# RaphaelHaddad/Real-Time-Brain-Inspired-Video-Memory

Measured on NVIDIA B200. Metric: queries_per_sec_top10_384d, higher is better.
Workload: dtype tf32

## Files before the change

### real-time-brain-inspired-video-memory_b200/csrc/common.cuh

```cuda
#pragma once
#include <cuda_runtime.h>
#include <cuda_bf16.h>
#include <stdint.h>
#include <stdio.h>
#include <math.h>
#include <utility>
#include "../../include/vidmem.h"

namespace vm {

void set_error(const char *fmt, ...);
#define VM_CUDA_CHECK(expr)                                                                      \
    do {                                                                                         \
        cudaError_t _e = (expr);                                                                 \
        if (_e != cudaSuccess) {                                                                 \
            vm::set_error("%s failed: %s (%s:%d)", #expr, cudaGetErrorString(_e), __FILE__, __LINE__); \
            return VM_ERR_CUDA;                                                                  \
        }                                                                                        \
    } while (0)
#define VM_REQUIRE(cond, code, ...)          \
    do {                                     \
        if (!(cond)) {                       \
            vm::set_error(__VA_ARGS__);      \
            return (code);                   \
        }                                    \
    } while (0)

__device__ __forceinline__ void pdl_wait() { asm volatile("griddepcontrol.wait;" ::: "memory"); }
__device__ __forceinline__ void pdl_launch_dependents() { asm volatile("griddepcontrol.launch_dependents;" ::: "memory"); }

template <typename... KArgs, typename... Args>
static inline cudaError_t launch_pdl(void (*kernel)(KArgs...), dim3 grid, dim3 block, size_t smem, cudaStream_t st, bool pdl,
                                     Args &&...args)
{
    cudaLaunchConfig_t cfg = {};
    cfg.gridDim = grid; cfg.blockDim = block; cfg.dynamicSmemBytes = smem; cfg.stream = st;
    cudaLaunchAttribute at[1];
    at[0].id = cudaLaunchAttributeProgrammaticStreamSerialization;
    at[0].val.programmaticStreamSerializationAllowed = 1;
    cfg.attrs = at;
    cfg.numAttrs = pdl ? 1 : 0;
    return cudaLaunchKernelEx(&cfg, kernel, std::forward<Args>(args)...);
}

template <auto Kernel>
static inline cudaError_t max_smem_once(int bytes)
{
    static bool set[64] = {};
    int dev = 0;
    cudaError_t e = cudaGetDevice(&dev);
    if (e != cudaSuccess || set[dev & 63]) return e;
    e = cudaFuncSetAttribute(Kernel, cudaFuncAttributeMaxDynamicSharedMemorySize, bytes);
    if (e == cudaSuccess) set[dev & 63] = true;
    return e;
}

__host__ __device__ __forceinline__ uint32_t f32_ordered(float f)
{
#ifdef __CUDA_ARCH__
    uint32_t b = __float_as_uint(f);
#else
    uint32_t b;
    memcpy(&b, &f, 4);
#endif
    return (b & 0x80000000u) ? ~b : (b | 0x80000000u);
}
__host__ __device__ __forceinline__ float f32_from_ordered(uint32_t o)
{
    uint32_t b = (o & 0x80000000u) ? (o & 0x7FFFFFFFu) : ~o;
#ifdef __CUDA_ARCH__
    return __uint_as_float(b);
#else
    float f;
    memcpy(&f, &b, 4);
    return f;
#endif
}
__host__ __device__ __forceinline__ uint64_t make_key(float score, uint32_t row)
{
    return ((uint64_t)f32_ordered(score) << 32) | (uint64_t)(0xFFFFFFFFu - row);
}
__host__ __device__ __forceinline__ uint32_t key_row(uint64_t k) { return 0xFFFFFFFFu - (uint32_t)(k & 0xFFFFFFFFu); }
// ... 210 lines not shown
```

### real-time-brain-inspired-video-memory_b200/csrc/scan_tc.cu

```cuda
#include "tc_common.cuh"

namespace vm {
using namespace tc;

static constexpr int TC_BLOCK_M = 128;
static constexpr int TC_STAGE_BYTES = TC_BLOCK_M * 128;
static constexpr int TC_ACC = 8;
static constexpr int TC_THREADS_SVC = 288;
static constexpr int TC_THREADS = 192;
static constexpr int TC_TMEM_COLS = 512;
static constexpr int TC_MAX_STAGES = 8;

struct CollectArgs {
    const float *thr;
    uint64_t *buf;
    int *cnt;
    int cap;
    const int *pending;
};

struct BandArgs {
    uint64_t *slab;
    int *scnt;
    uint64_t *ubuf;
// ... 15 lines not shown
    const int es = dtype == VM_F32 ? 4 : 2;
    L.nq_pad = (nq + 15) & ~15;
    L.KB = (ld * es + 127) / 128;
    L.split = (split && dtype == VM_BF16) ? 1 : 0;
    uint32_t o = 0;
    L.off_b = o; o += (uint32_t)L.KB * L.nq_pad * 128 * (L.split ? 2 : 1);
    const uint32_t epi = (uint32_t)L.nq_pad * (4 + 4 + 4 + 16) + 64 + 8 * (2 * TC_MAX_STAGES + 1 + 2 * TC_ACC) + 16;
    int64_t room = 227 * 1024 - 2048 - (int64_t)o - epi;
    L.stages = (int)(room / TC_STAGE_BYTES);
    if (L.stages > TC_MAX_STAGES) L.stages = TC_MAX_STAGES;
    if (L.stages < 0) L.stages = 0;
    L.off_a = o; o += (uint32_t)L.stages * TC_STAGE_BYTES;
    L.off_tauf = o; o += (uint32_t)L.nq_pad * 4;
    L.off_lcnt = o; o += (uint32_t)L.nq_pad * 4;
    L.off_cmax = o; o += (uint32_t)L.nq_pad * 4;
    L.off_wmax = o; o += (uint32_t)L.nq_pad * 16;
    L.off_flags = o; o += 64;
    L.off_bars = o; o += 8 * (2 * TC_MAX_STAGES + 1 + 2 * TC_ACC);
    L.off_tmem = o; o += 16;
    L.total = o + 1024;
#ifdef VIDMEM_AB_SMEMPAD
    if (L.total < 220 * 1024) L.total = 220 * 1024;
#endif
    return L;
}

__device__ __forceinline__ uint32_t own_kth_score(const uint64_t *slab, int n, int k, int lane)
{
    constexpr int PER = SCAN_SLAB / 32;
    uint32_t vals[PER];
#pragma unroll
    for (int t = 0; t < PER; ++t) {
        const int i = lane + 32 * t;
        vals[t] = i < n ? (uint32_t)(__ldcg(slab + i) >> 32) : 0u;
    }
    uint32_t prefix = 0;
    int need = k;
    for (int bit = 31; bit >= 12; --bit) {
        const uint32_t hi = bit == 31 ? 0u : (0xFFFFFFFFu << (bit + 1));
        int cnt = 0;
#pragma unroll
        for (int t = 0; t < PER; ++t) cnt += ((vals[t] & hi) == prefix && ((vals[t] >> bit) & 1u)) ? 1 : 0;
        const int tot = __reduce_add_sync(0xffffffffu, cnt);
        if (tot >= need) prefix |= 1u << bit;
        else need -= tot;
    }
    int ge = 0;
#pragma unroll
    for (int t = 0; t < PER; ++t) ge += (vals[t] != 0u && vals[t] >= prefix) ? 1 : 0;
    ge = __reduce_add_sync(0xffffffffu, ge);
    return (ge >= k && prefix != 0u) ? prefix : 0u;
}

template <bool TF32, bool DUMP, bool SPLIT>
__global__ void __launch_bounds__(DUMP ? TC_THREADS : TC_THREADS_SVC, 1)
scan_tc_kernel(const __grid_constant__ CUtensorMap tmA, const __grid_constant__ CUtensorMap tmB,
               const float *__restrict__ inv_norms, int64_t n, int num_tiles, int nq, TcLayout L, uint64_t *__restrict__ dump_keys,
               uint32_t *__restrict__ seed_tab, int *__restrict__ seed_ctr, CollectArgs col, BandArgs ub, int svc_sleep)
{
    const bool collect = !DUMP && col.thr != nullptr;
#ifndef VIDMEM_AB_NOPDL
    pdl_launch_dependents();
#endif
    if (collect) {
        pdl_wait();
        if (*col.pending == 0) return;
    }

    extern __shared__ __align__(16) uint8_t smem_raw[];
    uint8_t *base = smem_raw + ((1024u - (smem_u32(smem_raw) & 1023u)) & 1023u);
    uint8_t *sB = base + L.off_b;
    uint8_t *sA = base + L.off_a;
    float *tauf = (float *)(base + L.off_tauf);
    int *lcnt = (int *)(base + L.off_lcnt);
    uint32_t *cmax = (uint32_t *)(base + L.off_cmax);
    uint32_t *wmax = (uint32_t *)(base + L.off_wmax);
    volatile int *s_done = (volatile int *)(base + L.off_flags);
    uint64_t *bars = (uint64_t *)(base + L.off_bars);
    uint64_t *full = bars, *empty = bars + TC_MAX_STAGES, *qfull = bars + 2 * TC_MAX_STAGES;
    uint64_t *tfull = qfull + 1, *tempty = tfull + TC_ACC;
    uint32_t *tmem_slot = (uint32_t *)(base + L.off_tmem);

    const int warp = __shfl_sync(0xffffffffu, threadIdx.x >> 5, 0);
    const int lane = threadIdx.x & 31;
    const int nq_pad = L.nq_pad, KB = L.KB, stages = L.stages;
    constexpr int ELEMS = TF32 ? 32 : 64;

    if (warp == 0 && lane == 0) {
        tma_prefetch_desc(&tmA);
        tma_prefetch_desc(&tmB);
        for (int s = 0; s < stages; ++s) { mbar_init(&full[s], 1); mbar_init(&empty[s], 1); }
        mbar_init(qfull, 1);
        for (int a = 0; a < TC_ACC; ++a) { mbar_init(&tfull[a], 1); mbar_init(&tempty[a], 4); }
        fence_barrier_init();
    }
    if (warp == 1) tmem_alloc(tmem_slot, TC_TMEM_COLS);
#ifndef VIDMEM_AB_NOPDL
    if (!collect) pdl_wait();
#endif
    if (warp >= 2 && warp < 6) {
        const int e = threadIdx.x - 64;
        if (e < nq_pad) {
            lcnt[e] = 0;
            cmax[e] = 0u;
            tauf[e] = collect ? (e < nq ? col.thr[e] : INFINITY) : (e < nq ? -INFINITY : INFINITY);
        }
        if (e < 2) s_done[e] = 0;
    }
    tc_fence_before();
    __syncthreads();
    tc_fence_after();
    const uint32_t tmem_base = *tmem_slot;
    uint32_t *gbound = seed_tab ? seed_tab + SEED_TAB_WORDS : nullptr;

    if (warp == 0) {
        if (elect_one()) {
            constexpr int QPARTS = SPLIT ? 2 : 1;
            mbar_arrive_expect_tx(qfull, (uint32_t)(KB * QPARTS) * nq_pad * 128);
            for (int part = 0; part < QPARTS; ++part)
                for (int kb = 0; kb < KB; ++kb)
                    tma_load_2d(&tmB, qfull, sB + (size_t)(part * KB + kb) * nq_pad * 128, kb * ELEMS, part * nq_pad, L2_EVICT_LAST);
        }
        __syncwarp();
        int stage = 0;
        uint32_t phase = 0;
        for (int tile = blockIdx.x; tile < num_tiles; tile += gridDim.x) {
            for (int kb = 0; kb < KB; ++kb) {
                mbar_wait(&empty[stage], phase ^ 1);
                if (elect_one()) {
                    mbar_arrive_expect_tx(&full[stage], TC_STAGE_BYTES);
                    tma_load_2d(&tmA, &full[stage], sA + (size_t)stage * TC_STAGE_BYTES, kb * ELEMS, tile * TC_BLOCK_M, L2_EVICT_FIRST);
                }
                __syncwarp();
                if (++stage == stages) { stage = 0; phase ^= 1; }
            }
        }
    } else if (warp == 1) {
        const uint32_t idesc = make_idesc(TF32 ? 2u : 1u, TC_BLOCK_M, (uint32_t)nq_pad);
        mbar_wait(qfull, 0);
        tc_fence_after();
        int stage = 0, acc = 0;
        uint32_t phase = 0, acc_phase = 0;
        const uint64_t da0 = make_smem_desc_sw128(smem_u32(sA)), db0 = make_smem_desc_sw128(smem_u32(sB));
        const uint32_t kb_step = (uint32_t)(nq_pad * 128) >> 4, lo_step = (uint32_t)(KB * nq_pad * 128) >> 4;
        for (int tile = blockIdx.x; tile < num_tiles; tile += gridDim.x) {
            mbar_wait(&tempty[acc], acc_phase ^ 1);
            tc_fence_after();
            const uint32_t d_tmem = tmem_base + (uint32_t)(acc * nq_pad);
            for (int kb = 0; kb < KB; ++kb) {
                mbar_wait(&full[stage], phase);
                tc_fence_after();
                if (elect_one()) {
                    const uint64_t da = da0 + (uint64_t)((uint32_t)stage * (TC_STAGE_BYTES >> 4));
                    const uint64_t db = db0 + (uint64_t)((uint32_t)kb * kb_step);
#pragma unroll
                    for (int j = 0; j < 4; ++j) {
                        umma<TF32>(d_tmem, da + 2 * j, db + 2 * j, idesc, (uint32_t)((kb | j) != 0));
                        if constexpr (SPLIT) umma<TF32>(d_tmem, da + 2 * j, db + lo_step + 2 * j, idesc, 1u);
                    }
                    umma_commit(&empty[stage]);
                    if (kb == KB - 1) umma_commit(&tfull[acc]);
                }
                __syncwarp();
                if (++stage == stages) { stage = 0; phase ^= 1; }
            }
            if (++acc == TC_ACC) { acc = 0; acc_phase ^= 1; }
        }
    } else if (warp < 6) {
        const int e = threadIdx.x - 64;
        const int quad = warp & 3;
        const int row_in_tile = quad * 32 + lane;
        int acc = 0;
        uint32_t acc_phase = 0;
        if constexpr (DUMP) {
            for (int tile = blockIdx.x; tile < num_tiles; tile += gridDim.x) {
                const int64_t r = (int64_t)tile * TC_BLOCK_M + row_in_tile;
                const float iv = r < n ? __ldg(inv_norms + r) : -1.0f;
                mbar_wait(&tfull[acc], acc_phase);
                tc_fence_after();
                const uint32_t taddr = tmem_base + ((uint32_t)(quad * 32) << 16) + (uint32_t)(acc * nq_pad);
                uint64_t *out = dump_keys + (int64_t)tile * nq * TC_BLOCK_M + row_in_tile;
                for (int c = 0; c < nq_pad; c += 16) {
                    uint32_t v[16];
                    tmem_ld16(taddr + c, v);
                    tmem_ld_wait();
#pragma unroll
                    for (int j = 0; j < 16; ++j)
                        if (c + j < nq)
                            out[(int64_t)(c + j) * TC_BLOCK_M] = iv >= 0.0f ? make_key(__uint_as_float(v[j]) * iv, (uint32_t)r) : 0ull;
                }
                tc_fence_before();
                __syncwarp();
                if (lane == 0) mbar_arrive(&tempty[acc]);
                if (++acc == TC_ACC) { acc = 0; acc_phase ^= 1; }
            }
        } else {
        if (ub.use_seed && !collect) {
            const int64_t row0 = (int64_t)blockIdx.x * TC_BLOCK_M + row_in_tile;
            const float inv0 = row0 < n ? __ldg(inv_norms + row0) : -1.0f;
            mbar_wait(&tfull[0], 0);
            tc_fence_after();
            const uint32_t taddr0 = tmem_base + ((uint32_t)(quad * 32) << 16);
            for (int c = 0; c < nq_pad; c += 16) {
                uint32_t v[16];
                tmem_ld16(taddr0 + c, v);
// ... 87 lines not shown
                            if (key == 1) tauf[q] = 0.0f;
                            continue;
#endif
                            const int pos = atomicAdd(&lcnt[q], 1);
                            atomicMax(&cmax[q], (uint32_t)(key >> 32));
                            if (pos < SCAN_SLAB) __stcg(my_slab + (size_t)q * SCAN_SLAB + pos, key);
                            else {
                                const int p = atomicAdd(ub.ucnt + q, 1);
                                if (p < ub.ucap) __stcg(ub.ubuf + (size_t)q * ub.ucap + p, key);
                                else tauf[q] = INFINITY;
                            }
                        }
                    }
                }
            };
            uint32_t va[16], vb[16];
#ifdef VIDMEM_AB_NOEPI
            if (tile < 0)
#endif
            tmem_ld16(taddr, va);
#ifdef VIDMEM_AB_NOEPI
            if (tile < 0)
#endif
            for (int c = 0; c < nq_pad; c += 32) {
                tmem_ld_wait();
                if (c + 16 < nq_pad) tmem_ld16(taddr + c + 16, vb);
                process(va, c);
                if (c + 16 < nq_pad) {
                    tmem_ld_wait();
                    if (c + 32 < nq_pad) tmem_ld16(taddr + c + 32, va);
                    process(vb, c + 16);
                }
            }
#ifdef VIDMEM_AB_TILEBAR
            named_bar_sync(1, 128);
#endif
            tc_fence_before();
            __syncwarp();
            if (lane == 0) mbar_arrive(&tempty[acc]);
            if (++acc == TC_ACC) { acc = 0; acc_phase ^= 1; }
            row = row_next;
            inv = inv_next;
        }
        if (!collect) {
            named_bar_sync(1, 128);
            if (e < nq) {
                ub.scnt[(size_t)blockIdx.x * nq + e] = lcnt[e];
                if (seed_tab != nullptr) __stcg(seed_tab + (size_t)blockIdx.x * nq_pad + e, cmax[e]);
            }
        }
        }
        __syncwarp();
        if (lane == 0) atomicAdd((int *)s_done, 1);
    } else {
#ifdef VIDMEM_AB_NOSVC
        if (false) {
#else
        if (!DUMP && warp == 8 && seed_tab != nullptr && !collect) {
#endif
            const int G = (int)gridDim.x;
            while (s_done[1] == 0 && s_done[0] < 4) __nanosleep(100);
            uint32_t pub0 = 0xFFFFFFFFu, pub1 = 0xFFFFFFFFu;
            uint32_t kth_done = 0;
            const uint64_t *my_slab = ub.slab + (size_t)blockIdx.x * nq * SCAN_SLAB;
            while (!__any_sync(0xffffffffu, s_done[0] >= 4)) {
#pragma unroll
                for (int h = 0; h < 2; ++h) {
                    const int q = lane + 32 * h;
                    if (q < nq) {
                        const uint32_t c = *(volatile uint32_t *)(cmax + q);
                        uint32_t &pub = h ? pub1 : pub0;
                        if (c != pub && c != 0u) { __stcg(seed_tab + (size_t)blockIdx.x * nq_pad + q, c); pub = c; }
                    }
                }
                __syncwarp();
                if (G >= ub.ksel)
                    for (int q = blockIdx.x; q < nq; q += G) {
                        const float sd = seed_select(seed_tab, G, nq_pad, q, ub.ksel, lane);
                        if (lane == 0 && sd > -INFINITY) atomicMax(gbound + q, f32_ordered(sd));
                    }
                __syncwarp();
#ifndef VIDMEM_AB_KTH_LEVELS
#define VIDMEM_AB_KTH_LEVELS 2
#endif
#ifndef VIDMEM_AB_KTH_PER_ROUND
#define VIDMEM_AB_KTH_PER_ROUND 1
#endif
                {
                    constexpr int LV = VIDMEM_AB_KTH_LEVELS;
                    int served = 0;
#pragma unroll
                    for (int h = 0; h < 2; ++h) {
                        const int q = lane + 32 * h;
                        int level = 0;
                        if (q < nq) {
                            const int have = *(volatile int *)(lcnt + q);
#pragma unroll
                            for (int l = 1; l <= LV; ++l) level = have >= (SCAN_SLAB >> (LV - l)) ? l : level;
                        }
                        const int done = (int)((kth_done >> (4 * h)) & 15u);
                        unsigned todo = __ballot_sync(0xffffffffu, level > done && (SCAN_SLAB >> (LV - level)) >= ub.ksel);
                        while (todo && (VIDMEM_AB_KTH_PER_ROUND == 0 || served < VIDMEM_AB_KTH_PER_ROUND)) {
                            const int src = __ffs(todo) - 1;
                            todo &= todo - 1;
                            ++served;
                            const int lv = __shfl_sync(0xffffffffu, level, src);
                            const int qq = src + 32 * h;
                            const uint32_t ok = own_kth_score(my_slab + (size_t)qq * SCAN_SLAB, SCAN_SLAB >> (LV - lv), ub.ksel, lane);
                            if (lane == src && ok != 0u) {
                                atomicMax(gbound + qq, ok);
                                kth_done = (kth_done & ~(15u << (4 * h))) | ((uint32_t)lv << (4 * h));
                            }
                        }
                    }
                }
                __syncwarp();
#pragma unroll
                for (int h = 0; h < 2; ++h) {
                    const int q = lane + 32 * h;
                    if (q < nq) {
                        const uint32_t o = __ldcg(gbound + q);
                        if (o != 0u) {
                            const float f = band_floor(f32_from_ordered(o), ub.band);
                            if (f > tauf[q]) *(volatile float *)(tauf + q) = f;
                        }
                    }
                }
                __nanosleep(svc_sleep);
            }
        }
    }

    tc_fence_before();
    __syncthreads();
    if (warp == 1) {
        tc_fence_after();
        tmem_dealloc(tmem_base, TC_TMEM_COLS);
    }
}

bool scan_tc_supported(int dtype, int dim, int nq, int kp, int split)
{
    (void)kp;
    if (dtype != VM_F32 && dtype != VM_BF16) return false;
    if (nq < 1 || nq > 64) return false;
    TcLayout L = make_layout(dtype, ld_for_dim(dim), nq, split);
    return L.stages >= 3;
}

int launch_scan_tc(const ScanArgs &a, const void *queries_store_dtype, uint32_t *seed_tab, int *seed_ctr, const ScanCollect *sc,
                   ScanInfo *info)
{
    VM_REQUIRE(a.n >= 1 && a.n < 0x7FFFFF00LL, VM_ERR_UNSUPPORTED, "tcgen05 scan: shard rows %lld outside [1, 2^31)", (long long)a.n);
    TcLayout L = make_layout(a.dtype, a.ld, a.nq, a.split);
    VM_REQUIRE(L.stages >= 3, VM_ERR_UNSUPPORTED, "tcgen05 scan: dim %d x %d queries does not fit shared memory", a.dim, a.nq);
    CUtensorMap tmA, tmB;
    int rc = make_tmap_2d_cached(&tmA, a.rows, a.dtype, (uint64_t)a.n, (uint64_t)a.ld, (uint64_t)a.ld, TC_BLOCK_M);
    if (rc != VM_OK) return rc;
    rc = make_tmap_2d_cached(&tmB, queries_store_dtype, a.dtype, (uint64_t)L.nq_pad * (L.split ? 2 : 1), (uint64_t)a.ld, (uint64_t)a.ld,
                             (uint32_t)L.nq_pad);
    if (rc != VM_OK) return rc;
    const int num_tiles = (int)((a.n + TC_BLOCK_M - 1) / TC_BLOCK_M);
    const bool dump = a.dump && !sc;
    if (sc || dump || a.ctas > 256) { seed_tab = nullptr; seed_ctr = nullptr; }
    CollectArgs col{};
    if (sc) { col.thr = sc->thr; col.buf = sc->buf; col.cnt = sc->cnt; col.cap = sc->cap; col.pending = sc->pending; }
    BandArgs ub{a.slab, a.scnt, a.ubuf, a.ucnt, a.ucap, a.band, a.ksel, 0};
    ub.use_seed = (seed_tab && seed_ctr && a.ksel >= 1 && a.ctas >= a.ksel) ? 1 : 0;
    if (!sc && !dump)
        VM_REQUIRE(ub.slab && ub.scnt && ub.ubuf && ub.ucnt && ub.ucap > 0 && ub.ksel >= 1, VM_ERR_BADARG, "tcgen05 scan: slab / spill buffers missing");
    if (dump) VM_REQUIRE(TC_BLOCK_M == SCAN_DUMP_TILE && (int64_t)num_tiles * TC_BLOCK_M <= SCAN_DUMP_MAX_KEYS && a.ctas == num_tiles,
                         VM_ERR_UNSUPPORTED, "tcgen05 scan: dump mode needs one CTA per tile and at most %d rows", SCAN_DUMP_MAX_KEYS);
#ifdef VIDMEM_AB_SVCSLEEP
    const int svc_sleep = VIDMEM_AB_SVCSLEEP;
#else
    const int svc_sleep = a.dtype == VM_F32 ? 500 : 200;
#endif
    if (info && !sc) { info->stages = L.stages; info->variant = dump ? 1 : 2; }
    const bool pdl = a.pdl && !sc;
#ifdef VIDMEM_AB_CLASSIC_LAUNCH
#define LAUNCH_IMPL(TF, DU, SP) scan_tc_kernel<TF, DU, SP><<<a.ctas, DU ? TC_THREADS : TC_THREADS_SVC, L.total, a.stream>>>(tmA, tmB, a.inv_norms, a.n, num_tiles, a.nq, L, a.cand, seed_tab, seed_ctr, col, ub, svc_sleep)
#else
#define LAUNCH_IMPL(TF, DU, SP) VM_CUDA_CHECK(launch_pdl(scan_tc_kernel<TF, DU, SP>, dim3(a.ctas), dim3(DU ? TC_THREADS : TC_THREADS_SVC), L.total, a.stream, pdl, \
                                 tmA, tmB, a.inv_norms, a.n, num_tiles, a.nq, L, a.cand, seed_tab, seed_ctr, col, ub, svc_sleep))
#endif
#define LAUNCH_TC(TF, DU, SP)                                                                                                \
    do {                                                                                                                   \
        VM_CUDA_CHECK((max_smem_once<scan_tc_kernel<TF, DU, SP>>(227 * 1024)));                                              \
        LAUNCH_IMPL(TF, DU, SP);                                                                                           \
    } while (0)
    if (a.dtype == VM_F32) { if (dump) LAUNCH_TC(true, true, false); else LAUNCH_TC(true, false, false); }
    else if (L.split) { if (dump) LAUNCH_TC(false, true, true); else LAUNCH_TC(false, false, true); }
// ... 9 lines not shown
```

### real-time-brain-inspired-video-memory_b200/csrc/select.cu

```cuda
#include "common.cuh"

#include <type_traits>

namespace vm {

static constexpr int MERGE_THREADS = 512;
static constexpr int MERGE_SURV = 1024;

__device__ uint64_t radix_select_kth(const uint64_t *skeys, int total, int kp, int *hist, int *s_bin, int *s_need)
{
    const int tid = threadIdx.x, lane = tid & 31;
    uint64_t prefix = 0;
    int need = kp;
    for (int pass = 0; pass < 8; ++pass) {
        const int shift = 56 - 8 * pass;
        const uint64_t hmask = pass == 0 ? 0ull : (~0ull << (shift + 8));
        if (tid < 256) hist[tid] = 0;
        __syncthreads();
        for (int e = tid; e < total; e += MERGE_THREADS) {
            const uint64_t k = skeys[e];
            const bool act = k != 0 && (k & hmask) == prefix;
            const int bin = act ? (int)((k >> shift) & 0xFF) : -1;
            const unsigned peers = __match_any_sync(__activemask(), bin);
            if (act && (__ffs(peers) - 1) == lane) atomicAdd(&hist[bin], __popc(peers));
// ... 405 lines not shown
        cp_async_commit();
    }
    const int kind = j < kp ? 0 : (j < 2 * kp ? 1 : ((j == 2 * kp && s_qq != nullptr) ? 2 : 3));
    const int cidx = kind == 0 ? j : (kind == 1 ? j - kp : 0);
    const bool active = kind == 2 || (kind < 2 && s_rid[cidx] != NO_ROW);
    const T *mine = reinterpret_cast<const T *>(srow + (size_t)cidx * pitch);
    constexpr int EPG = 16 / (int)sizeof(T);
    RefSum acc;
    acc.init();
#pragma unroll
    for (int c = 0; c < 3; ++c) {
        if (c == 0) cp_async_wait<2>();
        else if (c == 1) cp_async_wait<1>();
        else cp_async_wait<0>();
        __syncthreads();
        const int g_lo = c == 0 ? 0 : (c == 1 ? c1 : c2), g_hi = c == 0 ? c1 : (c == 1 ? c2 : gpr);
        const int i_lo = g_lo * EPG, i_hi = min(g_hi * EPG, dim);
        if (active) {
            if (kind == 0)
                ref_sum_range<NEUMAIER>(acc, i_lo, i_hi, [&](int i) { return __dmul_rn(sq[i], load_elem(mine, i)); });
            else if (kind == 1)
                ref_sum_range<NEUMAIER>(acc, i_lo, i_hi, [&](int i) { const double y = load_elem(mine, i); return __dmul_rn(y, y); });
            else
                ref_sum_range<NEUMAIER>(acc, i_lo, i_hi, [&](int i) { const double x = sq[i]; return __dmul_rn(x, x); });
        }
    }
    if (active) {
        const double r = acc.result<NEUMAIER>();
        if (kind == 0) s_dot[cidx] = r;
        else if (kind == 1) s_rr[cidx] = r;
        else *s_qq = r;
    }
    __syncthreads();
}

struct SelectSrc {
    const uint64_t *cand;
    int lists, list_len;
    int complete;
    const uint64_t *slab;
    const int *scnt;
    int ctas;
    const uint64_t *ubuf;
    const int *ucnt;
    int ucap;
    const uint32_t *seed_tab;
    int nq_pad, ksel;
    float band;
    int key_cap;
    int band_cap;
};

template <int THREADS>
__device__ int load_slab_keys(const SelectSrc &src, int q, int nq, uint64_t *skeys, int *s_cnts, int *s_total, float *s_bf, bool *incomplete)
{
    const int tid = threadIdx.x, lane = tid & 31, warp = tid >> 5;
    if (warp == 0) {
        float Lb = -INFINITY;
        if (src.seed_tab != nullptr) {
            if (src.ctas >= src.ksel) Lb = seed_select(src.seed_tab, src.ctas, src.nq_pad, q, src.ksel, lane);
            const uint32_t o = __ldcg(src.seed_tab + SEED_TAB_WORDS + q);
            if (o != 0u) Lb = fmaxf(Lb, f32_from_ordered(o));
        }
        if (lane == 0) { *s_bf = band_floor(Lb, src.band); *s_total = 0; }
    }
    for (int c = tid; c < src.ctas; c += THREADS) s_cnts[c] = min(src.scnt[(size_t)c * nq + q], SCAN_SLAB);
    __syncthreads();
    const float bf = *s_bf;
    constexpr int WARPS = THREADS / 32, PER = SCAN_SLAB / 32, BATCH = 4;
    for (int c0 = warp; c0 < src.ctas; c0 += WARPS * BATCH) {
        uint64_t kk[BATCH][PER];
#pragma unroll
        for (int b = 0; b < BATCH; ++b) {
            const int c = c0 + b * WARPS;
            const int cnt = c < src.ctas ? s_cnts[c] : 0;
#pragma unroll
            for (int t = 0; t < PER; ++t)
                kk[b][t] = (lane + 32 * t < cnt) ? __ldcg(src.slab + ((size_t)c * nq + q) * SCAN_SLAB + lane + 32 * t) : 0ull;
        }
#pragma unroll
        for (int b = 0; b < BATCH; ++b)
#pragma unroll
            for (int t = 0; t < PER; ++t) {
                const uint64_t k = kk[b][t];
                if (k != 0 && key_score(k) >= bf) {
                    const int p = atomicAdd(s_total, 1);
                    if (p < src.key_cap) skeys[p] = k;
                }
            }
    }
    const int spilled = src.ucnt[q];
    const int ns = min(spilled, src.ucap);
    for (int e = tid; e < ns; e += THREADS) {
        const uint64_t k = __ldcg(src.ubuf + (size_t)q * src.ucap + e);
        if (k != 0 && key_score(k) >= bf) {
            const int p = atomicAdd(s_total, 1);
            if (p < src.key_cap) skeys[p] = k;
        }
    }
    __syncthreads();
    const int got = *s_total;
    *incomplete = spilled > src.ucap || got > src.key_cap;
    return min(got, src.key_cap);
}

__global__ void __launch_bounds__(SR_THREADS) slab_top_kernel(SelectSrc src, int nq, int kp, uint64_t *__restrict__ merged,
                                                             int *__restrict__ incomplete)
{
    extern __shared__ __align__(16) unsigned char st_smem[];
    uint64_t *skeys = reinterpret_cast<uint64_t *>(st_smem);
    __shared__ int s_cnts[256];
    __shared__ int s_total, s_bin, s_need, s_m;
    __shared__ int hist[256];
    __shared__ float s_bf;
    const int q = blockIdx.x, tid = threadIdx.x;
    bool inc = false;
    const int total = load_slab_keys<SR_THREADS>(src, q, nq, skeys, s_cnts, &s_total, &s_bf, &inc);
    for (int e = tid; e < kp; e += SR_THREADS) merged[(int64_t)q * kp + e] = 0;
    if (tid == 0) { incomplete[q] = inc ? 1 : 0; s_m = 0; }
    __syncthreads();
    if (total <= MERGE_SURV) {
        for (int e = tid; e < total; e += SR_THREADS) {
            const uint64_t k = skeys[e];
            int rank = 0;
            for (int i = 0; i < total; ++i) rank += skeys[i] > k ? 1 : 0;
            if (rank < kp) merged[(int64_t)q * kp + rank] = k;
        }
        return;
    }
    const uint64_t Tk = radix_select_kth(skeys, total, kp, hist, &s_bin, &s_need);
    for (int e = tid; e < total; e += SR_THREADS) {
        const uint64_t k = skeys[e];
        if (k > Tk) merged[(int64_t)q * kp + atomicAdd(&s_m, 1)] = k;
        else if (k == Tk) merged[(int64_t)q * kp + kp - 1] = k;
    }
}

template <bool NEUMAIER, typename T>
__global__ void __launch_bounds__(SR_THREADS, 1) select_rescore_kernel(SelectSrc src, int nq, int kp,
                                                                   const T *__restrict__ rows, int ld, int dim, int64_t n_rows,
                                                                   const void *__restrict__ queries, int q_dtype, double eps,
                                                                   FinalizeArgs f, int32_t *__restrict__ flags,
                                                                   int32_t *__restrict__ uncertified_count,
                                                                   const int *__restrict__ extreme, float *__restrict__ collect_thr,
                                                                   unsigned long long *__restrict__ cum, const float *__restrict__ inv_norms)
{
    extern __shared__ __align__(16) unsigned char sr_smem[];
    uint64_t *skeys = reinterpret_cast<uint64_t *>(sr_smem);
    uint32_t *lmax = reinterpret_cast<uint32_t *>(skeys + src.key_cap);
    double *sq = reinterpret_cast<double *>(lmax + ((src.lists + 3) & ~3));
    const int pitch = ld * (int)sizeof(T) + 16;
    unsigned char *srow = reinterpret_cast<unsigned char *>(sq + ((dim + 1) & ~1));
    double *b_sc = reinterpret_cast<double *>(srow + (((size_t)kp * pitch + 15) & ~(size_t)15));
    uint32_t *b_row = reinterpret_cast<uint32_t *>(b_sc + src.band_cap);
    __shared__ uint64_t s_top[64];
    __shared__ uint32_t s_rid[64];
    __shared__ uint64_t surv[MERGE_SURV];
    __shared__ int hist[256];
    __shared__ int s_bin, s_need, s_m, s_nz, s_cnt, s_band, s_viol, s_out, s_total;
    __shared__ int s_cnts[256];
    __shared__ uint32_t s_L;
    __shared__ float s_thr, s_bf;
    __shared__ double s_dot[64], s_rr[64], s_qq, s_score[64];
    const int q = blockIdx.x, tid = threadIdx.x, lane = tid & 31, warp = tid >> 5;

    pdl_launch_dependents();
    if (tid == 0) { s_m = 0; s_nz = 0; s_cnt = 0; s_band = 0; s_viol = 0; s_thr = -INFINITY; }
    if (tid < 64) s_top[tid] = 0;
    pdl_wait();
    __syncthreads();

    const bool union_mode = src.slab != nullptr;
    int total, lists = src.lists, list_len = src.list_len;
    bool overflow = false;
    int nz = 0;
    if (union_mode) {
        total = load_slab_keys<SR_THREADS>(src, q, nq, skeys, s_cnts, &s_total, &s_bf, &overflow);
        lists = 0;
        if (tid == 0) nz = total;
    } else {
        total = lists * list_len;
#pragma unroll 10
        for (int e = tid; e < total; e += SR_THREADS) {
            const int l = e / list_len, j = e - l * list_len;
            const uint64_t k = src.cand[((int64_t)l * nq + q) * list_len + j];
            skeys[e] = k;
            nz += k != 0;
        }
    }
    for (int i = tid; i < dim; i += SR_THREADS) sq[i] = load_as_double(queries, q_dtype, (int64_t)q * dim + i);
    if (nz) atomicAdd(&s_nz, nz);
    __syncthreads();
    const int nonzero = s_nz;
    bool done = false;
    if (total <= MERGE_SURV) {
        for (int e = tid; e < total; e += SR_THREADS) {
            const uint64_t k = skeys[e];
            if (k == 0) continue;
            int rank = 0;
            for (int i = 0; i < total; ++i) rank += skeys[i] > k ? 1 : 0;
            if (rank < kp) s_top[rank] = k;
        }
        done = true;
    } else if (nonzero >= kp && lists >= kp && lists <= 256) {
        for (int l = warp; l < lists; l += SR_THREADS / 32) {
            uint32_t m = 0;
            for (int j = lane; j < list_len; j += 32) m = max(m, (uint32_t)(skeys[l * list_len + j] >> 32));
            m = __reduce_max_sync(0xffffffffu, m);
            if (lane == 0) lmax[l] = m;
        }
        __syncthreads();
        if (warp == 0) {
            uint32_t vals[8];
#pragma unroll
            for (int t = 0; t < 8; ++t) vals[t] = (lane + 32 * t) < lists ? lmax[lane + 32 * t] : 0u;
            uint32_t prefix = 0;
            int need = kp;
            for (int bit = 31; bit >= 12; --bit) {
                const uint32_t hi = bit == 31 ? 0u : (0xFFFFFFFFu << (bit + 1));
                int cnt = 0;
#pragma unroll
                for (int t = 0; t < 8; ++t) cnt += ((vals[t] & hi) == prefix && ((vals[t] >> bit) & 1u)) ? 1 : 0;
                const int tot = __reduce_add_sync(0xffffffffu, cnt);
                if (tot >= need) prefix |= 1u << bit;
                else need -= tot;
            }
            if (lane == 0) s_L = prefix;
        }
        __syncthreads();
        const uint32_t Lb = s_L;
        if (Lb != 0) {
            for (int e = tid; e < total; e += SR_THREADS) {
                const uint64_t k = skeys[e];
                if ((uint32_t)(k >> 32) >= Lb && k != 0) {
                    const int p = atomicAdd(&s_m, 1);
                    if (p < MERGE_SURV) surv[p] = k;
                }
            }
            __syncthreads();
            const int m = s_m;
            if (m >= kp && m <= MERGE_SURV) {
                for (int e = tid; e < m; e += SR_THREADS) {
                    const uint64_t k = surv[e];
                    int rank = 0;
                    for (int i = 0; i < m; ++i) rank += surv[i] > k ? 1 : 0;
                    if (rank < kp) s_top[rank] = k;
                }
                done = true;
            }
        }
    }
    if (!done) {
        __syncthreads();
        uint64_t Tk = 1;
        if (nonzero >= kp) Tk = radix_select_kth(skeys, total, kp, hist, &s_bin, &s_need);
        if (tid == 0) s_m = 0;
        __syncthreads();
        for (int e = tid; e < total; e += SR_THREADS) {
            const uint64_t k = skeys[e];
            if (k >= Tk && k != 0) {
                if (nonzero >= kp && k == Tk) s_top[kp - 1] = k;
                else s_top[atomicAdd(&s_m, 1)] = k;
            }
        }
    }
    __syncthreads();

    const int j = tid;
    const uint64_t mykey = j < 64 ? s_top[j] : 0;
    const bool cand_valid = j < kp && mykey != 0;
    if (j < 64) s_rid[j] = cand_valid ? key_row(mykey) : NO_ROW;
    __syncthreads();
    stage_and_chain<NEUMAIER, T, SR_THREADS>(rows, ld, dim, kp, s_rid, srow, pitch, sq, s_dot, s_rr, &s_qq);

    double sc = 0.0;
    const uint32_t row = cand_valid ? key_row(mykey) : 0;
    const double n1 = __dsqrt_rn(s_qq);
    if (n1 == 0.0) {
        if (tid == 0) {
            int c = 0;
            const double outv = convert_score(0.0, f.score_mode);
            if (outv > f.min_score)
                for (int64_t r = 0; r < n_rows && c < f.k; ++r)
                    if (__ldg(inv_norms + r) >= 0.0f) {
                        f.out_idx[(int64_t)q * f.k + c] = r + f.row_offset;
                        f.out_score[(int64_t)q * f.k + c] = outv;
                        ++c;
                    }
            for (int t = c; t < f.k; ++t) { f.out_idx[(int64_t)q * f.k + t] = -1; f.out_score[(int64_t)q * f.k + t] = 0.0; }
            f.out_count[q] = c;
            flags[q] = 0;
            if (collect_thr) collect_thr[q] = INFINITY;
        }
        return;
    }
    if (cand_valid) {
        const double n2 = __dsqrt_rn(s_rr[j]);
        sc = (n1 == 0.0 || n2 == 0.0) ? 0.0 : __ddiv_rn(s_dot[j], __dmul_rn(n1, n2));
        if (fabs((double)key_score(mykey) - sc) > eps) atomicAdd(&s_viol, 1);
    }
    if (j < 64) s_score[j] = sc;
    __syncthreads();
    int ncand = 0;
    for (int i = 0; i < kp; ++i) ncand += s_top[i] != 0;
    int rank = 0;
    if (cand_valid)
        for (int i = 0; i < kp; ++i)
            if (s_top[i] != 0 && i != j && better(s_score[i], key_row(s_top[i]), sc, row)) ++rank;
    const double outv = convert_score(sc, f.score_mode);
    const bool emit = cand_valid && rank < f.k && outv > f.min_score;
    if (emit) {
        f.out_idx[(int64_t)q * f.k + rank] = (int64_t)row + f.row_offset;
        f.out_score[(int64_t)q * f.k + rank] = outv;
        atomicAdd(&s_cnt, 1);
    }
    if (cand_valid && ncand >= f.k && rank == f.k - 1) {
        float t = (float)(sc - eps);
        t = nextafterf(nextafterf(t, -INFINITY), -INFINITY);
        s_thr = t;
    }
    __syncthreads();
    const float thr = s_thr;
    {
        int inb = 0;
        for (int e = tid; e < total; e += SR_THREADS) {
            const uint64_t k = skeys[e];
            inb += (k != 0 && key_score(k) >= thr) ? 1 : 0;
        }
        if (inb) atomicAdd(&s_band, inb);
    }
    __syncthreads();
    const int band = s_band;
    const bool bound_ok = !(extreme && *extreme != 0) && s_viol == 0;
    const bool src_complete = union_mode ? !overflow : (src.complete != 0);
    bool cert;
    if (src_complete) cert = band <= ncand;
    else if (union_mode) cert = false;
    else cert = ncand < kp || band < kp;
    if (!bound_ok && (int64_t)ncand < n_rows) cert = false;
    if (ncand == 0) cert = true;
    if (cert) {
        if (tid == 0) {
            flags[q] = 0;
            if (collect_thr) collect_thr[q] = INFINITY;
            f.out_count[q] = s_cnt;
        }
        const int cnt = s_cnt;
        for (int t = cnt + tid; t < f.k; t += SR_THREADS) {
            f.out_idx[(int64_t)q * f.k + t] = -1;
            f.out_score[(int64_t)q * f.k + t] = 0.0;
        }
        return;
    }
    if (tid == 0 && cum) { atomicAdd(cum, 1ull); if (s_viol) atomicAdd(cum + 4, 1ull); }
    if (bound_ok && src_complete && band <= src.band_cap) {
        if (tid == 0) s_m = 0;
        __syncthreads();
        for (int e = tid; e < total; e += SR_THREADS) {
            const uint64_t k = skeys[e];
            if (k != 0 && key_score(k) >= thr) b_row[atomicAdd(&s_m, 1)] = key_row(k);
        }
        __syncthreads();
        for (int b0 = 0; b0 < band; b0 += kp) {
            const int cnt = min(kp, band - b0);
            if (tid < 64) s_rid[tid] = tid < cnt ? b_row[b0 + tid] : NO_ROW;
            __syncthreads();
            stage_and_chain<NEUMAIER, T, SR_THREADS>(rows, ld, dim, kp, s_rid, srow, pitch, sq, s_dot, s_rr, nullptr);
            if (tid < cnt) {
                const double n2 = __dsqrt_rn(s_rr[tid]);
                b_sc[b0 + tid] = (n1 == 0.0 || n2 == 0.0) ? 0.0 : __ddiv_rn(s_dot[tid], __dmul_rn(n1, n2));
            }
            __syncthreads();
        }
        band_emit<SR_THREADS>(band, b_sc, b_row, &s_out, f, q);
        if (tid == 0) {
            flags[q] = 0;
            if (collect_thr) collect_thr[q] = INFINITY;
            if (cum) atomicAdd(cum + 1, 1ull);
        }
        return;
    }
    if (tid == 0) {
        flags[q] = bound_ok ? 1 : 2;
        if (collect_thr) {
            float t = thr > -INFINITY ? (float)((double)thr - eps) : -INFINITY;
            t = nextafterf(t, -INFINITY);
            collect_thr[q] = bound_ok ? t : INFINITY;
        }
        atomicAdd(uncertified_count, 1);
        f.out_count[q] = s_cnt;
    }
    const int cnt = s_cnt;
    for (int t = cnt + tid; t < f.k; t += SR_THREADS) {
        f.out_idx[(int64_t)q * f.k + t] = -1;
        f.out_score[(int64_t)q * f.k + t] = 0.0;
    }
}

static constexpr int CR_THREADS = 512;
template <bool NEUMAIER, typename T>
__global__ void __launch_bounds__(CR_THREADS, 1) collect_rescore_kernel(const uint64_t *__restrict__ buf, const int *__restrict__ cnt, int cap,
                                                                       const T *__restrict__ rows, int ld, int dim,
                                                                       const void *__restrict__ queries, int q_dtype, FinalizeArgs f,
                                                                       int32_t *__restrict__ flags, int32_t *__restrict__ uncertified_count,
                                                                       int nq, unsigned long long *__restrict__ cum, int stage_rows)
{
    extern __shared__ __align__(16) unsigned char cr_smem[];
    double *sq = reinterpret_cast<double *>(cr_smem);
    double *s_sc = sq + ((dim + 1) & ~1);
    double *s_rr = s_sc + cap;
    uint32_t *s_row = reinterpret_cast<uint32_t *>(s_sc + (stage_rows > 0 ? cap : 2 * cap));
    const int pitch = ld * (int)sizeof(T) + 16;
    unsigned char *srow = reinterpret_cast<unsigned char *>(s_row + ((cap + 3) & ~3));
    __shared__ double s_n1;
    __shared__ int s_out;
    __shared__ uint32_t s_rid[64];
    __shared__ double s_dot[64], s_r2[64];
    const int q = blockIdx.x, tid = threadIdx.x;
    if (flags[nq] == 0 || flags[q] != 1) return;
    const int m = cnt[q];
    if (m > cap) {
        if (tid == 0) flags[q] = 2;
        return;
    }
    for (int i = tid; i < dim; i += CR_THREADS) sq[i] = load_as_double(queries, q_dtype, (int64_t)q * dim + i);
    for (int e = tid; e < m; e += CR_THREADS) s_row[e] = key_row(buf[(size_t)q * cap + e]);
    __syncthreads();
// ... 616 lines not shown
```

### real-time-brain-inspired-video-memory_b200/csrc/store.cu

```cuda
#include "common.cuh"
#include "synth.cuh"

namespace vm {

template <typename DST>
__global__ void convert_rows_kernel(const void *__restrict__ src, int src_dtype, DST *__restrict__ dst, int64_t n,
                                    int dim, int ld)
{
    int64_t total = n * (int64_t)ld;
    for (int64_t e = blockIdx.x * (int64_t)blockDim.x + threadIdx.x; e < total; e += (int64_t)gridDim.x * blockDim.x) {
        int64_t r = e / ld;
        int c = (int)(e - r * ld);
        double dv = 0.0;
        if (c < dim) dv = load_as_double(src, src_dtype, r * dim + c);
        if constexpr (sizeof(DST) == 8) dst[e] = dv;
        else {
            const float v = (float)dv;
            if constexpr (sizeof(DST) == 4) dst[e] = v;
            else dst[e] = __float2bfloat16_rn(v);
        }
    }
}

template <typename T>
__global__ void row_inv_norms_kernel(const T *__restrict__ rows, float *__restrict__ inv_norms, int64_t row0,
                                     int64_t n, int ld, int *__restrict__ extreme, const double *__restrict__ exact)
{
    int lane = threadIdx.x & 31;
    int64_t warp = (blockIdx.x * (int64_t)blockDim.x + threadIdx.x) >> 5;
    int64_t nwarps = ((int64_t)gridDim.x * blockDim.x) >> 5;
    for (int64_t r = row0 + warp; r < n; r += nwarps) {
        const T *p = rows + r * (int64_t)ld;
        double ss = 0.0;
        for (int c = lane; c < ld; c += 32) {
            double v = (double)load_as_float(p, c);
            ss += v * v;
        }
        for (int o = 16; o > 0; o >>= 1) ss += __shfl_xor_sync(0xffffffffu, ss, o);
        double se = 0.0;
        if (exact != nullptr) {
            for (int c = lane; c < ld; c += 32) {
                const double v = exact[r * (int64_t)ld + c] * 0x1p-600;
                se += v * v;
            }
            for (int o = 16; o > 0; o >>= 1) se += __shfl_xor_sync(0xffffffffu, se, o);
        }
        if (lane == 0) {
            float inv = 0.0f;
            if (!isfinite(ss)) {
                inv = -1.0f;
                if (exact != nullptr && isfinite(se)) { inv = 0.0f; if (extreme) atomicAdd(extreme, 1); }
            } else if (ss > 0.0) {
                inv = (float)(1.0 / sqrt(ss));
                if (extreme && (ss < 7.52316384526264e-37 || ss > 1.329227995784916e+36)) atomicAdd(extreme, 1);
            } else if (exact != nullptr && se != 0.0) {
                if (extreme) atomicAdd(extreme, 1);
            }
            inv_norms[r] = inv;
        }
    }
}

__global__ void invalidate_rows_kernel(float *inv_norms, const int64_t *rows, int64_t n, int64_t size)
{
    int64_t i = blockIdx.x * (int64_t)blockDim.x + threadIdx.x;
    if (i < n && rows[i] >= 0 && rows[i] < size) inv_norms[rows[i]] = -1.0f;
}

__global__ void normalize_queries_kernel(const void *__restrict__ q, int q_dtype, int nq, int nq_pad, int dim, int ld,
                                         float *__restrict__ out_f32, __nv_bfloat16 *__restrict__ out_bf16,
                                         int32_t *__restrict__ zero_me, uint32_t *__restrict__ zero_tab, int zero_tab_n,
                                         int tf32_round, int split)
{
    pdl_launch_dependents();
    pdl_wait();
    if (zero_me && blockIdx.x == 0 && threadIdx.x < 2) zero_me[threadIdx.x] = 0;
    for (int i = blockIdx.x * blockDim.x + threadIdx.x; i < zero_tab_n; i += gridDim.x * blockDim.x) zero_tab[i] = 0u;
    int lane = threadIdx.x & 31;
    int w = (blockIdx.x * blockDim.x + threadIdx.x) >> 5;
    if (w >= nq_pad) return;
    double ss = 0.0;
    if (w < nq)
        for (int c = lane; c < dim; c += 32) {
            double v = load_as_double(q, q_dtype, (int64_t)w * dim + c);
            ss += v * v;
        }
    for (int o = 16; o > 0; o >>= 1) ss += __shfl_xor_sync(0xffffffffu, ss, o);
    double inv = (ss > 0.0 && isfinite(ss)) ? 1.0 / sqrt(ss) : 0.0;
    for (int c = lane; c < ld; c += 32) {
        float v = 0.0f;
        if (w < nq && c < dim) v = (float)(load_as_double(q, q_dtype, (int64_t)w * dim + c) * inv);
        float vf = v;
        if (tf32_round) vf = __uint_as_float((__float_as_uint(v) + 0x1000u) & 0xFFFFE000u);
        out_f32[(int64_t)w * ld + c] = vf;
        if (out_bf16) {
            const __nv_bfloat16 hi = __float2bfloat16_rn(v);
            out_bf16[(int64_t)w * ld + c] = hi;
            if (split) out_bf16[((int64_t)nq_pad + w) * ld + c] = __float2bfloat16_rn(v - __bfloat162float(hi));
        }
    }
}

template <typename T>
__global__ void synth_fill_kernel(T *__restrict__ rows, uint64_t seed, int64_t row0, int64_t n, int dim, int ld,
                                  uint64_t dup_period)
{
    int groups = ld >> 3;
    int64_t total = n * (int64_t)groups;
    uint64_t hk = splitmix64(seed ^ 0xD6E8FEB86659FD93ULL);
    for (int64_t e = blockIdx.x * (int64_t)blockDim.x + threadIdx.x; e < total; e += (int64_t)gridDim.x * blockDim.x) {
        int64_t i = e / groups;
        int g = (int)(e - i * groups);
        uint64_t row = (uint64_t)(row0 + i);
        uint64_t own = splitmix64(splitmix64(seed * 0x9E3779B97F4A7C15ULL + row) + (uint64_t)g);
        uint64_t par = 0, sel = 0;
        bool planted = false;
        if (dup_period > 0 && row > 0) {
            uint64_t hr = splitmix64(hk + row);
            if (hr % dup_period == 0) {
                planted = true;
                uint64_t parent = splitmix64(hr) % row;
                par = splitmix64(splitmix64(seed * 0x9E3779B97F4A7C15ULL + parent) + (uint64_t)g);
                sel = splitmix64(hr + 0x632BE59BD9B4E019ULL + (uint64_t)g);
            }
        }
        T *dst = rows + i * (int64_t)ld + g * 8;
#pragma unroll
        for (int b = 0; b < 8; ++b) {
            int col = g * 8 + b;
            int v = synth_int(own, b);
            if (planted && (((sel >> (8 * b)) & 15ULL) != 0ULL)) v = synth_int(par, b);
            float f = col < dim ? (float)v * (1.0f / 128.0f) : 0.0f;
            if constexpr (sizeof(T) == 4) dst[b] = f;
            else dst[b] = __float2bfloat16_rn(f);
        }
    }
}

int k_convert_rows(const void *src, int src_dtype, void *dst, int dst_dtype, int64_t n, int dim, int ld, cudaStream_t st)
{
    if (n <= 0) return VM_OK;
    int64_t total = n * (int64_t)ld;
    int grid = (int)vm::imin64((total + 255) / 256, 148 * 16);
    if (dst_dtype == VM_F32) convert_rows_kernel<float><<<grid, 256, 0, st>>>(src, src_dtype, (float *)dst, n, dim, ld);
    else if (dst_dtype == VM_F64) convert_rows_kernel<double><<<grid, 256, 0, st>>>(src, src_dtype, (double *)dst, n, dim, ld);
    else convert_rows_kernel<__nv_bfloat16><<<grid, 256, 0, st>>>(src, src_dtype, (__nv_bfloat16 *)dst, n, dim, ld);
    VM_CUDA_CHECK(cudaGetLastError());
    return VM_OK;
}

int k_row_inv_norms(const void *rows, int dtype, float *inv_norms, int64_t row0, int64_t n, int ld, int *extreme, cudaStream_t st,
                    const double *exact)
{
// ... 43 lines not shown
```

Before: 260,000.

## Hoist pre-PDL prologue work and batch slab key loads ahead of sync

The scan kernel's producer warp now issues the first pipeline stages of row-tile TMA loads before the PDL wait, so they overlap the previous kernel's tail. The select kernel loads query rows and the first batch of slab keys and counts into registers before the barrier, with a larger batch and without the shared count array. The query normalization kernel computes norms from register-cached values before the PDL wait. Optional globaltimer probes are added behind a compile flag. The larger register batches may raise register pressure, and issuing row loads before the wait assumes the row data is not written by the preceding kernel.

Measured after the change: 261,100, median of 6. About the same (+0.4%).

```diff
diff --git a/real-time-brain-inspired-video-memory_b200/csrc/common.cuh b/real-time-brain-inspired-video-memory_b200/csrc/common.cuh
--- a/real-time-brain-inspired-video-memory_b200/csrc/common.cuh
+++ b/real-time-brain-inspired-video-memory_b200/csrc/common.cuh
@@ -28,6 +28,21 @@
 
 __device__ __forceinline__ void pdl_wait() { asm volatile("griddepcontrol.wait;" ::: "memory"); }
 __device__ __forceinline__ void pdl_launch_dependents() { asm volatile("griddepcontrol.launch_dependents;" ::: "memory"); }
+
+#ifdef VIDMEM_PHASE_PROBE
+static constexpr int PROBE_SCAN_SLOTS = 3;
+static constexpr int PROBE_SEL_SLOTS = 5;
+static constexpr int PROBE_MAX_CTAS = 256, PROBE_MAX_Q = 64;
+__device__ __forceinline__ unsigned long long probe_now()
+{
+    unsigned long long t;
+    asm volatile("mov.u64 %0, %%globaltimer;" : "=l"(t));
+    return t;
+}
+#define VM_PROBE(tab, slot) ((tab)[slot] = probe_now())
+#else
+#define VM_PROBE(tab, slot) ((void)0)
+#endif
 
 template <typename... KArgs, typename... Args>
 static inline cudaError_t launch_pdl(void (*kernel)(KArgs...), dim3 grid, dim3 block, size_t smem, cudaStream_t st, bool pdl,
diff --git a/real-time-brain-inspired-video-memory_b200/csrc/scan_tc.cu b/real-time-brain-inspired-video-memory_b200/csrc/scan_tc.cu
--- a/real-time-brain-inspired-video-memory_b200/csrc/scan_tc.cu
+++ b/real-time-brain-inspired-video-memory_b200/csrc/scan_tc.cu
@@ -91,6 +91,10 @@
     return (ge >= k && prefix != 0u) ? prefix : 0u;
 }
 
+#ifdef VIDMEM_PHASE_PROBE
+__device__ unsigned long long g_probe_scan[PROBE_MAX_CTAS * PROBE_SCAN_SLOTS];
+#endif
+
 template <bool TF32, bool DUMP, bool SPLIT>
 __global__ void __launch_bounds__(DUMP ? TC_THREADS : TC_THREADS_SVC, 1)
 scan_tc_kernel(const __grid_constant__ CUtensorMap tmA, const __grid_constant__ CUtensorMap tmB,
@@ -125,13 +129,30 @@
     const int nq_pad = L.nq_pad, KB = L.KB, stages = L.stages;
     constexpr int ELEMS = TF32 ? 32 : 64;
 
-    if (warp == 0 && lane == 0) {
-        tma_prefetch_desc(&tmA);
-        tma_prefetch_desc(&tmB);
-        for (int s = 0; s < stages; ++s) { mbar_init(&full[s], 1); mbar_init(&empty[s], 1); }
-        mbar_init(qfull, 1);
-        for (int a = 0; a < TC_ACC; ++a) { mbar_init(&tfull[a], 1); mbar_init(&tempty[a], 4); }
-        fence_barrier_init();
+    int p_stage = 0, p_tile = blockIdx.x, p_kb = 0;
+    uint32_t p_phase = 0;
+    if (warp == 0) {
+        if (lane == 0) {
+            tma_prefetch_desc(&tmA);
+            tma_prefetch_desc(&tmB);
+            for (int s = 0; s < stages; ++s) { mbar_init(&full[s], 1); mbar_init(&empty[s], 1); }
+            mbar_init(qfull, 1);
+            for (int a = 0; a < TC_ACC; ++a) { mbar_init(&tfull[a], 1); mbar_init(&tempty[a], 4); }
+            fence_barrier_init();
+        }
+        __syncwarp();
+        if (!collect) {
+            if (lane == 0) VM_PROBE(g_probe_scan, blockIdx.x * PROBE_SCAN_SLOTS + 0);
+            for (int s = 0; s < stages && p_tile < num_tiles; ++s) {
+                if (elect_one()) {
+                    mbar_arrive_expect_tx(&full[s], TC_STAGE_BYTES);
+                    tma_load_2d(&tmA, &full[s], sA + (size_t)s * TC_STAGE_BYTES, p_kb * ELEMS, p_tile * TC_BLOCK_M, L2_EVICT_FIRST);
+                }
+                __syncwarp();
+                if (++p_stage == stages) { p_stage = 0; p_phase ^= 1; }
+                if (++p_kb == KB) { p_kb = 0; p_tile += gridDim.x; }
+            }
+        }
     }
     if (warp == 1) tmem_alloc(tmem_slot, TC_TMEM_COLS);
 #ifndef VIDMEM_AB_NOPDL
@@ -161,10 +182,10 @@
                     tma_load_2d(&tmB, qfull, sB + (size_t)(part * KB + kb) * nq_pad * 128, kb * ELEMS, part * nq_pad, L2_EVICT_LAST);
         }
         __syncwarp();
-        int stage = 0;
-        uint32_t phase = 0;
-        for (int tile = blockIdx.x; tile < num_tiles; tile += gridDim.x) {
-            for (int kb = 0; kb < KB; ++kb) {
+        int stage = p_stage, kb = p_kb;
+        uint32_t phase = p_phase;
+        for (int tile = p_tile; tile < num_tiles; tile += gridDim.x, kb = 0) {
+            for (; kb < KB; ++kb) {
                 mbar_wait(&empty[stage], phase ^ 1);
                 if (elect_one()) {
                     mbar_arrive_expect_tx(&full[stage], TC_STAGE_BYTES);
@@ -190,6 +211,9 @@
                 mbar_wait(&full[stage], phase);
                 tc_fence_after();
                 if (elect_one()) {
+#ifdef VIDMEM_PHASE_PROBE
+                    if (tile == blockIdx.x && kb == 0 && !collect) VM_PROBE(g_probe_scan, blockIdx.x * PROBE_SCAN_SLOTS + 1);
+#endif
                     const uint64_t da = da0 + (uint64_t)((uint32_t)stage * (TC_STAGE_BYTES >> 4));
                     const uint64_t db = db0 + (uint64_t)((uint32_t)kb * kb_step);
 #pragma unroll
@@ -383,6 +407,9 @@
         }
         __syncwarp();
         if (lane == 0) atomicAdd((int *)s_done, 1);
+#ifdef VIDMEM_PHASE_PROBE
+        if (e == 0 && !collect) VM_PROBE(g_probe_scan, blockIdx.x * PROBE_SCAN_SLOTS + 2);
+#endif
     } else {
 #ifdef VIDMEM_AB_NOSVC
         if (false) {
@@ -469,6 +496,13 @@
         tmem_dealloc(tmem_base, TC_TMEM_COLS);
     }
 }
+
+#ifdef VIDMEM_PHASE_PROBE
+extern "C" int vm_probe_read_scan(unsigned long long *host)
+{
+    return cudaMemcpyFromSymbol(host, g_probe_scan, sizeof(g_probe_scan)) == cudaSuccess ? VM_OK : VM_ERR_CUDA;
+}
+#endif
 
 bool scan_tc_supported(int dtype, int dim, int nq, int kp, int split)
 {
diff --git a/real-time-brain-inspired-video-memory_b200/csrc/select.cu b/real-time-brain-inspired-video-memory_b200/csrc/select.cu
--- a/real-time-brain-inspired-video-memory_b200/csrc/select.cu
+++ b/real-time-brain-inspired-video-memory_b200/csrc/select.cu
@@ -481,9 +481,24 @@
 };
 
 template <int THREADS>
-__device__ int load_slab_keys(const SelectSrc &src, int q, int nq, uint64_t *skeys, int *s_cnts, int *s_total, float *s_bf, bool *incomplete)
+__device__ int load_slab_keys(const SelectSrc &src, int q, int nq, uint64_t *skeys, int *s_total, float *s_bf, bool *incomplete)
 {
     const int tid = threadIdx.x, lane = tid & 31, warp = tid >> 5;
+    constexpr int WARPS = THREADS / 32, PER = SCAN_SLAB / 32, BATCH = 10;
+    uint64_t kk[BATCH][PER];
+    int cnt[BATCH];
+    auto load = [&](int c0) {
+#pragma unroll
+        for (int b = 0; b < BATCH; ++b) {
+            const int c = c0 + b * WARPS;
+            const bool have = c < src.ctas;
+            cnt[b] = have ? __ldcg(src.scnt + (size_t)c * nq + q) : 0;
+#pragma unroll
+            for (int t = 0; t < PER; ++t) kk[b][t] = have ? __ldcg(src.slab + ((size_t)c * nq + q) * SCAN_SLAB + lane + 32 * t) : 0ull;
+        }
+    };
+    load(warp);
+    const int spilled = __ldcg(src.ucnt + q);
     if (warp == 0) {
         float Lb = -INFINITY;
         if (src.seed_tab != nullptr) {
@@ -493,32 +508,23 @@
         }
         if (lane == 0) { *s_bf = band_floor(Lb, src.band); *s_total = 0; }
     }
-    for (int c = tid; c < src.ctas; c += THREADS) s_cnts[c] = min(src.scnt[(size_t)c * nq + q], SCAN_SLAB);
     __syncthreads();
     const float bf = *s_bf;
-    constexpr int WARPS = THREADS / 32, PER = SCAN_SLAB / 32, BATCH = 4;
-    for (int c0 = warp; c0 < src.ctas; c0 += WARPS * BATCH) {
-        uint64_t kk[BATCH][PER];
-#pragma unroll
-        for (int b = 0; b < BATCH; ++b) {
-            const int c = c0 + b * WARPS;
-            const int cnt = c < src.ctas ? s_cnts[c] : 0;
-#pragma unroll
-            for (int t = 0; t < PER; ++t)
-                kk[b][t] = (lane + 32 * t < cnt) ? __ldcg(src.slab + ((size_t)c * nq + q) * SCAN_SLAB + lane + 32 * t) : 0ull;
-        }
+    for (int c0 = warp;;) {
 #pragma unroll
         for (int b = 0; b < BATCH; ++b)
 #pragma unroll
             for (int t = 0; t < PER; ++t) {
                 const uint64_t k = kk[b][t];
-                if (k != 0 && key_score(k) >= bf) {
+                if (lane + 32 * t < min(cnt[b], SCAN_SLAB) && k != 0 && key_score(k) >= bf) {
                     const int p = atomicAdd(s_total, 1);
                     if (p < src.key_cap) skeys[p] = k;
                 }
             }
-    }
-    const int spilled = src.ucnt[q];
+        c0 += WARPS * BATCH;
+        if (c0 >= src.ctas) break;
+        load(c0);
+    }
     const int ns = min(spilled, src.ucap);
     for (int e = tid; e < ns; e += THREADS) {
         const uint64_t k = __ldcg(src.ubuf + (size_t)q * src.ucap + e);
@@ -538,13 +544,12 @@
 {
     extern __shared__ __align__(16) unsigned char st_smem[];
     uint64_t *skeys = reinterpret_cast<uint64_t *>(st_smem);
-    __shared__ int s_cnts[256];
     __shared__ int s_total, s_bin, s_need, s_m;
     __shared__ int hist[256];
     __shared__ float s_bf;
     const int q = blockIdx.x, tid = threadIdx.x;
     bool inc = false;
-    const int total = load_slab_keys<SR_THREADS>(src, q, nq, skeys, s_cnts, &s_total, &s_bf, &inc);
+    const int total = load_slab_keys<SR_THREADS>(src, q, nq, skeys, &s_total, &s_bf, &inc);
     for (int e = tid; e < kp; e += SR_THREADS) merged[(int64_t)q * kp + e] = 0;
     if (tid == 0) { incomplete[q] = inc ? 1 : 0; s_m = 0; }
     __syncthreads();
@@ -564,6 +569,17 @@
         else if (k == Tk) merged[(int64_t)q * kp + kp - 1] = k;
     }
 }
+
+#ifdef VIDMEM_PHASE_PROBE
+__device__ unsigned long long g_probe_sel[PROBE_MAX_Q * PROBE_SEL_SLOTS];
+extern "C" int vm_probe_read_select(unsigned long long *host)
+{
+    return cudaMemcpyFromSymbol(host, g_probe_sel, sizeof(g_probe_sel)) == cudaSuccess ? VM_OK : VM_ERR_CUDA;
+}
+#define SEL_PROBE(slot) do { if (tid == 0 && q < PROBE_MAX_Q) VM_PROBE(g_probe_sel, q * PROBE_SEL_SLOTS + (slot)); } while (0)
+#else
+#define SEL_PROBE(slot) ((void)0)
+#endif
 
 template <bool NEUMAIER, typename T>
 __global__ void __launch_bounds__(SR_THREADS, 1) select_rescore_kernel(SelectSrc src, int nq, int kp,
@@ -587,7 +603,6 @@
     __shared__ uint64_t surv[MERGE_SURV];
     __shared__ int hist[256];
     __shared__ int s_bin, s_need, s_m, s_nz, s_cnt, s_band, s_viol, s_out, s_total;
-    __shared__ int s_cnts[256];
     __shared__ uint32_t s_L;
     __shared__ float s_thr, s_bf;
     __shared__ double s_dot[64], s_rr[64], s_qq, s_score[64];
@@ -596,15 +611,18 @@
     pdl_launch_dependents();
     if (tid == 0) { s_m = 0; s_nz = 0; s_cnt = 0; s_band = 0; s_viol = 0; s_thr = -INFINITY; }
     if (tid < 64) s_top[tid] = 0;
+    for (int i = tid; i < dim; i += SR_THREADS) sq[i] = load_as_double(queries, q_dtype, (int64_t)q * dim + i);
     pdl_wait();
     __syncthreads();
+    SEL_PROBE(0);
 
     const bool union_mode = src.slab != nullptr;
     int total, lists = src.lists, list_len = src.list_len;
     bool overflow = false;
     int nz = 0;
     if (union_mode) {
-        total = load_slab_keys<SR_THREADS>(src, q, nq, skeys, s_cnts, &s_total, &s_bf, &overflow);
+        total = load_slab_keys<SR_THREADS>(src, q, nq, skeys, &s_total, &s_bf, &overflow);
+        SEL_PROBE(1);
         lists = 0;
         if (tid == 0) nz = total;
     } else {
@@ -617,7 +635,6 @@
             nz += k != 0;
         }
     }
-    for (int i = tid; i < dim; i += SR_THREADS) sq[i] = load_as_double(queries, q_dtype, (int64_t)q * dim + i);
     if (nz) atomicAdd(&s_nz, nz);
     __syncthreads();
     const int nonzero = s_nz;
@@ -695,12 +712,14 @@
     }
     __syncthreads();
 
+    SEL_PROBE(2);
     const int j = tid;
     const uint64_t mykey = j < 64 ? s_top[j] : 0;
     const bool cand_valid = j < kp && mykey != 0;
     if (j < 64) s_rid[j] = cand_valid ? key_row(mykey) : NO_ROW;
     __syncthreads();
     stage_and_chain<NEUMAIER, T, SR_THREADS>(rows, ld, dim, kp, s_rid, srow, pitch, sq, s_dot, s_rr, &s_qq);
+    SEL_PROBE(3);
 
     double sc = 0.0;
     const uint32_t row = cand_valid ? key_row(mykey) : 0;
@@ -774,6 +793,7 @@
             if (collect_thr) collect_thr[q] = INFINITY;
             f.out_count[q] = s_cnt;
         }
+        SEL_PROBE(4);
         const int cnt = s_cnt;
         for (int t = cnt + tid; t < f.k; t += SR_THREADS) {
             f.out_idx[(int64_t)q * f.k + t] = -1;
@@ -802,6 +822,7 @@
             __syncthreads();
         }
         band_emit<SR_THREADS>(band, b_sc, b_row, &s_out, f, q);
+        SEL_PROBE(4);
         if (tid == 0) {
             flags[q] = 0;
             if (collect_thr) collect_thr[q] = INFINITY;
diff --git a/real-time-brain-inspired-video-memory_b200/csrc/store.cu b/real-time-brain-inspired-video-memory_b200/csrc/store.cu
--- a/real-time-brain-inspired-video-memory_b200/csrc/store.cu
+++ b/real-time-brain-inspired-video-memory_b200/csrc/store.cu
@@ -73,23 +73,35 @@
                                          int tf32_round, int split)
 {
     pdl_launch_dependents();
+    const int lane = threadIdx.x & 31;
+    const int w = (blockIdx.x * blockDim.x + threadIdx.x) >> 5;
+    const bool live = w < nq;
+    constexpr int NQ_REG = 16;
+    double x[NQ_REG];
+    double ss = 0.0;
+#pragma unroll
+    for (int t = 0; t < NQ_REG; ++t) {
+        const int c = lane + 32 * t;
+        x[t] = live && c < dim ? load_as_double(q, q_dtype, (int64_t)w * dim + c) : 0.0;
+    }
+#pragma unroll
+    for (int t = 0; t < NQ_REG; ++t)
+        if (live && lane + 32 * t < dim) ss += x[t] * x[t];
+    if (live)
+        for (int c = lane + 32 * NQ_REG; c < dim; c += 32) {
+            const double v = load_as_double(q, q_dtype, (int64_t)w * dim + c);
+            ss += v * v;
+        }
+    for (int o = 16; o > 0; o >>= 1) ss += __shfl_xor_sync(0xffffffffu, ss, o);
+    const double inv = (ss > 0.0 && isfinite(ss)) ? 1.0 / sqrt(ss) : 0.0;
+
     pdl_wait();
     if (zero_me && blockIdx.x == 0 && threadIdx.x < 2) zero_me[threadIdx.x] = 0;
     for (int i = blockIdx.x * blockDim.x + threadIdx.x; i < zero_tab_n; i += gridDim.x * blockDim.x) zero_tab[i] = 0u;
-    int lane = threadIdx.x & 31;
-    int w = (blockIdx.x * blockDim.x + threadIdx.x) >> 5;
     if (w >= nq_pad) return;
-    double ss = 0.0;
-    if (w < nq)
-        for (int c = lane; c < dim; c += 32) {
-            double v = load_as_double(q, q_dtype, (int64_t)w * dim + c);
-            ss += v * v;
-        }
-    for (int o = 16; o > 0; o >>= 1) ss += __shfl_xor_sync(0xffffffffu, ss, o);
-    double inv = (ss > 0.0 && isfinite(ss)) ? 1.0 / sqrt(ss) : 0.0;
-    for (int c = lane; c < ld; c += 32) {
+    auto emit = [&](int c, double xc) {
         float v = 0.0f;
-        if (w < nq && c < dim) v = (float)(load_as_double(q, q_dtype, (int64_t)w * dim + c) * inv);
+        if (live && c < dim) v = (float)(xc * inv);
         float vf = v;
         if (tf32_round) vf = __uint_as_float((__float_as_uint(v) + 0x1000u) & 0xFFFFE000u);
         out_f32[(int64_t)w * ld + c] = vf;
@@ -98,7 +110,11 @@
             out_bf16[(int64_t)w * ld + c] = hi;
             if (split) out_bf16[((int64_t)nq_pad + w) * ld + c] = __float2bfloat16_rn(v - __bfloat162float(hi));
         }
-    }
+    };
+#pragma unroll
+    for (int t = 0; t < NQ_REG; ++t)
+        if (lane + 32 * t < ld) emit(lane + 32 * t, x[t]);
+    for (int c = lane + 32 * NQ_REG; c < ld; c += 32) emit(c, live && c < dim ? load_as_double(q, q_dtype, (int64_t)w * dim + c) : 0.0);
 }
 
 template <typename T>
```
